# AI4Science-WestlakeU/RealPDEBench

Measured on AMD Instinct MI355X. Metric: train-step samples/sec (+ autoregressive rollout fields/sec in 'rollout'), FNO cylinder 128^2, higher is better.
Workload: dtype f32 storage / split-bf16x3 MFMA contractions (six bf16 products per fp32 product, fp32 accumulate), fp32-grade

## Files before the change

### realpdebench_amd/csrc/rpb_pjg.hip

```cpp
#include "rpb_pjf.h"
#include "rpb_mma.h"
#include <stdlib.h>

#define PG_HID 128
#define PG_WAVES 4
#define PG_GH_PLANE 2048
#define PG_GH_BUF (3 * PG_GH_PLANE)
#define PG_GH_WAVE (2 * PG_GH_BUF)
#ifndef PG_PIPE1
#define PG_PIPE1 2
#endif

#ifdef PG_TIMING
#define PG_T(i)                                    \
    {                                              \
        __builtin_amdgcn_sched_barrier(0);         \
        const long long now_ = clock64();          \
        __builtin_amdgcn_sched_barrier(0);         \
        tacc[i] += (float)(now_ - tlast);          \
        tlast = now_;                              \
    }
#else
#define PG_T(i)
#endif

#define PG_MAC6(NC, ACC, AH, AM, AL, BH, BM, BL) PG_MAC6F(NC, ACC, AH, AM, AL, BH, BM, BL, PG_NOTFIRST)
#define PG_NOTFIRST(c) false
#define PG_MAC6F(NC, ACC, AH, AM, AL, BH, BM, BL, FIRST)                               \
    _Pragma("unroll") for (int c_ = 0; c_ < NC; ++c_) ACC(c_) = mfma32b(AH(c_), BL(c_), FIRST(c_) ? f32x16{} : ACC(c_)); \
    _Pragma("unroll") for (int c_ = 0; c_ < NC; ++c_) ACC(c_) = mfma32b(AL(c_), BH(c_), ACC(c_)); \
    _Pragma("unroll") for (int c_ = 0; c_ < NC; ++c_) ACC(c_) = mfma32b(AM(c_), BM(c_), ACC(c_)); \
    _Pragma("unroll") for (int c_ = 0; c_ < NC; ++c_) ACC(c_) = mfma32b(AH(c_), BM(c_), ACC(c_)); \
    _Pragma("unroll") for (int c_ = 0; c_ < NC; ++c_) ACC(c_) = mfma32b(AM(c_), BH(c_), ACC(c_)); \
    _Pragma("unroll") for (int c_ = 0; c_ < NC; ++c_) ACC(c_) = mfma32b(AH(c_), BH(c_), ACC(c_));

template <bool LOSS>
__global__ __launch_bounds__(PG_WAVES * 64, 1) void pjg_kernel(PjfArgs p) {
    extern __shared__ u32x4 lds4[];
    u32x4* W1B = lds4;
    u32x4* W1D = W1B + 4 * 4 * 3 * 64;
    float* b1l = reinterpret_cast<float*>(W1D + 8 * 2 * 3 * 64);
    float* meanl = b1l + PG_HID;
    float* gball = meanl + 64;
    char* GHall = reinterpret_cast<char*>(gball + PG_WAVES * 64);
    const int tid = threadIdx.x, lane = tid & 63;
    const int wave = __builtin_amdgcn_readfirstlane(tid >> 6);
    const int n = lane & 31, hg = lane >> 5;
    for (int idx = tid; idx < 4 * 4 * 64; idx += blockDim.x) {
        const int l = idx & 63, nt = (idx >> 6) & 3, ks = idx >> 8;
        float v[8];
#pragma unroll
        for (int e = 0; e < 8; ++e) {
            const int c = 16 * ks + 8 * (l >> 5) + e;
            v[e] = p.w1[(32 * nt + (l & 31)) * 64 + c] * (p.xf.gamma[c] * p.xf.invstd[c]);
        }
        bf16x8 h, m, lo;
        split8(v, h, m, lo);
        W1B[((ks * 4 + nt) * 3 + 0) * 64 + l] = __builtin_bit_cast(u32x4, h);
        W1B[((ks * 4 + nt) * 3 + 1) * 64 + l] = __builtin_bit_cast(u32x4, m);
        W1B[((ks * 4 + nt) * 3 + 2) * 64 + l] = __builtin_bit_cast(u32x4, lo);
    }
    for (int idx = tid; idx < 8 * 2 * 64; idx += blockDim.x) {
        const int l = idx & 63, mt = (idx >> 6) & 1, ks3 = idx >> 7;
        float v[8];
#pragma unroll
        for (int e = 0; e < 8; ++e) v[e] = p.w1[(16 * ks3 + 8 * (l >> 5) + e) * 64 + 32 * mt + (l & 31)];
        bf16x8 h, m, lo;
        split8(v, h, m, lo);
        W1D[((ks3 * 2 + mt) * 3 + 0) * 64 + l] = __builtin_bit_cast(u32x4, h);
        W1D[((ks3 * 2 + mt) * 3 + 1) * 64 + l] = __builtin_bit_cast(u32x4, m);
        W1D[((ks3 * 2 + mt) * 3 + 2) * 64 + l] = __builtin_bit_cast(u32x4, lo);
    }
    for (int h = tid; h < PG_HID; h += blockDim.x) {
        float a = p.b1[h];
        for (int c = 0; c < 64; ++c) a = __builtin_fmaf(p.w1[h * 64 + c], p.xf.beta[c], a);
        b1l[h] = a;
    }
    if (tid < 64) meanl[tid] = p.xf.mean[tid];
    __syncthreads();

    const CropMap cm = p.cm;
    const long nslots = (long)gridDim.x * PG_WAVES;
    const long slot = (long)blockIdx.x * PG_WAVES + wave;
    const unsigned line_bytes = (unsigned)cm.Wp * 256u;
    const f32x4 z4 = {0.f, 0.f, 0.f, 0.f};

    {
        const long G = (long)p.B * cm.Tp * cm.Hp;
        for (long g = slot; g < G; g += nslots) {
            const int h = (int)(g % cm.Hp);
            const int t = (int)((g / cm.Hp) % cm.Tp);
            if (h < cm.H && t < cm.T) continue;
            const rsrc_t ro = make_rsrc(p.g + g * cm.Wp * 64, line_bytes);
            for (int off = lane * 16; off < (int)line_bytes; off += 1024) st16<0>(z4, ro, off);
        }
    }

    const long GL = (long)p.B * cm.T * cm.H;
    const int TQ = (cm.W + 31) >> 5;
    char* GHw = GHall + wave * PG_GH_WAVE;
    float* gb = gball + wave * 64;
    const float meanB0 = p.xf.mean[2 * n], meanB1 = p.xf.mean[2 * n + 1];
    float w2r[2][4], b1r[4];
#pragma unroll
    for (int nt = 0; nt < 4; ++nt) {
        b1r[nt] = b1l[32 * nt + n];
        w2r[0][nt] = p.w2[32 * nt + n];
        w2r[1][nt] = p.w2[PG_HID + 32 * nt + n];
    }
    const float b2y = LOSS ? p.b2[n & 1] : 0.f;
    const int celly = 8 * (n >> 3) + 4 * hg + ((n >> 1) & 3);
    const int cells = 8 * ((n >> 2) & 3) + 4 * (n >> 4) + (n & 3);
    const int ghw0 = n * 64 + (((2 * hg + 0) ^ ((n >> 1) & 3)) << 4), ghw1 = n * 64 + (((2 * hg + 1) ^ ((n >> 1) & 3)) << 4);
    int tro[2];
    {
        const int s16 = lane & 15, a = s16 >> 2, b = s16 & 3, gsel = (lane >> 4) & 1;
#pragma unroll
        for (int hf = 0; hf < 2; ++hf) {
            const int row = 8 * hg + 4 * hf + a;
            tro[hf] = row * 64 + (((2 * gsel + (b >> 1)) ^ ((row >> 1) & 3)) << 4) + (b & 1) * 8;
        }
    }
    const bool bit3 = (n >> 3) & 1, bit2 = (n >> 2) & 1, bit1 = (n >> 1) & 1, bit0 = n & 1;

    float dw2[2][4], db1[4], gacc = 0.f, lacc = 0.f;
    f32x16 accM[4][2];
#pragma unroll
    for (int t = 0; t < 4; ++t) {
        db1[t] = 0.f;
        dw2[0][t] = dw2[1][t] = 0.f;
#pragma unroll
        for (int c = 0; c < 2; ++c)
#pragma unroll
            for (int r = 0; r < 16; ++r) accM[t][c][r] = 0.f;
    }

    auto line_of = [&](int gl) {
        const unsigned h = (unsigned)gl % (unsigned)cm.H, r2 = (unsigned)gl / (unsigned)cm.H;
        return (int)(((r2 / (unsigned)cm.T) * cm.Tp + r2 % (unsigned)cm.T) * cm.Hp + h);
    };
    u32x4 xa[8];
    auto issue_xa = [&](int pl, int q) {
        const bool ok = pl >= 0;
        const rsrc_t rx = make_rsrc(p.s + (long)(ok ? pl : 0) * cm.Wp * 64, ok ? (unsigned)cm.W * 256u : 0u);
#pragma unroll
        for (int i = 0; i < 8; ++i) xa[i] = ld16<0>(rx, (32 * q + n) * 256 + (i >> 1) * 64 + hg * 32 + (i & 1) * 16);
    };
    auto prefetch = [&](int pl, int q) -> unsigned {
        const bool ok = pl >= 0;
        const rsrc_t rx = make_rsrc(p.s + (long)(ok ? pl : 0) * cm.Wp * 64, ok ? (unsigned)cm.W * 256u : 0u);
        return __builtin_amdgcn_raw_buffer_load_b32(rx, 32 * q * 256 + lane * 128, 0, 0);
    };
    issue_xa(slot < GL ? line_of((int)slot) : -1, 0);
#ifdef PG_TIMING
    float tacc[12];
#pragma unroll
    for (int i = 0; i < 12; ++i) tacc[i] = 0.f;
    long long tlast = clock64();
#endif
    for (long gl = slot; gl < GL; gl += nslots) {
        const int pl = line_of((int)gl);
        const int gln = gl + nslots < GL ? (int)(gl + nslots) : -1;
        const int pln = gln >= 0 ? line_of(gln) : -1;
        const rsrc_t ro = make_rsrc(p.g + (long)pl * cm.Wp * 64, line_bytes);
        const rsrc_t rxl = make_rsrc(p.s + (long)pl * cm.Wp * 64, (unsigned)cm.W * 256u);
        const rsrc_t rg = make_rsrc(p.gout + gl * cm.W * 2, (unsigned)cm.W * 8u);
        for (int q = 0; q < TQ; ++q) {
            asm volatile("" ::: "memory");
            const bool last = q + 1 == TQ;
            const int pn = last ? pln : pl, qn = last ? 0 : q + 1;
            const unsigned pf = prefetch(pn, qn);
            const float yv = buf_load_f32(rg, ((32 * q + celly) * 2 + (n & 1)) * 4, 0);
            f32x4 G4[8];
            if (!LOSS) {
#pragma unroll
                for (int k = 0; k < 8; ++k) G4[k] = __builtin_bit_cast(f32x4, ld16<0>(rg, (32 * q + 8 * (k >> 1) + 4 * hg + 2 * (k & 1)) * 8));
            }
            PG_T(0)
            f32x16 acc[4];
#pragma unroll
            for (int nt = 0; nt < 4; ++nt)
#pragma unroll
                for (int r = 0; r < 16; ++r) acc[nt][r] = 0.f;
            bf16x8 Ah[2], Am[2], Al[2], bh[2][4], bm[2][4], bl[2][4];
            auto prep = [&](int ks) {
                float v[8];
                const f32x4 x0 = __builtin_bit_cast(f32x4, xa[2 * ks]), x1 = __builtin_bit_cast(f32x4, xa[2 * ks + 1]);
                const f32x4 m0 = *reinterpret_cast<const f32x4*>(meanl + 16 * ks + 8 * hg), m1 = *reinterpret_cast<const f32x4*>(meanl + 16 * ks + 8 * hg + 4);
#pragma unroll
                for (int c = 0; c < 4; ++c) {
                    v[c] = x0[c] - m0[c];
                    v[4 + c] = x1[c] - m1[c];
                }
                split8(v, Ah[ks & 1], Am[ks & 1], Al[ks & 1]);
#pragma unroll
                for (int nt = 0; nt < 4; ++nt) {
                    bh[ks & 1][nt] = __builtin_bit_cast(bf16x8, W1B[((ks * 4 + nt) * 3 + 0) * 64 + lane]);
                    bm[ks & 1][nt] = __builtin_bit_cast(bf16x8, W1B[((ks * 4 + nt) * 3 + 1) * 64 + lane]);
                    bl[ks & 1][nt] = __builtin_bit_cast(bf16x8, W1B[((ks * 4 + nt) * 3 + 2) * 64 + lane]);
                }
            };
            prep(0);
#pragma unroll
            for (int ks = 0; ks < 4; ++ks) {
                if (ks < 3) prep(ks + 1);
#define PG_ACC(c) acc[c]
#define PG_AH(c) Ah[ks & 1]
#define PG_AM(c) Am[ks & 1]
#define PG_AL(c) Al[ks & 1]
#define PG_BH(c) bh[ks & 1][c]
#define PG_BM(c) bm[ks & 1][c]
#define PG_BL(c) bl[ks & 1][c]
#define PG_FIRST(c) (ks == 0)
                PG_MAC6F(4, PG_ACC, PG_AH, PG_AM, PG_AL, PG_BH, PG_BM, PG_BL, PG_FIRST)
#undef PG_FIRST
#undef PG_ACC
#undef PG_AH
#undef PG_AM
#undef PG_AL
#undef PG_BH
#undef PG_BM
#undef PG_BL
#if PG_PIPE1
                if (ks < 3) {
#pragma unroll
                    for (int i = 0; i < 24; ++i) {
                        __builtin_amdgcn_sched_group_barrier(0x008, 1, 0);
                        __builtin_amdgcn_sched_group_barrier(0x002, PG_PIPE1, 0);
                        if (i < 14) __builtin_amdgcn_sched_group_barrier(0x100, 1, 0);
                    }
                }
                __builtin_amdgcn_sched_barrier(0);
#endif
            }
            asm volatile("" ::"v"(pf));
            __builtin_amdgcn_sched_barrier(0);
            PG_T(1)
            f32x2 xr[16];
            auto issue_xr = [&]() {
#pragma unroll
                for (int i = 0; i < 16; ++i) xr[i] = ld8<0>(rxl, (32 * q + 16 * (i >> 3) + 8 * ((i >> 2) & 1) + 4 * hg + (i & 3)) * 256 + n * 8);
            };
            float VV[4][16];
            if (LOSS) {
                f32x2 pp[16];
#pragma unroll
                for (int i = 0; i < 16; ++i) pp[i] = pk2(0.f);
#pragma unroll
                for (int nt = 0; nt < 4; ++nt) {
                    const f32x2 wp = {w2r[0][nt], w2r[1][nt]};
#pragma unroll
                    for (int r = 0; r < 16; r += 4) {
                        f32x2 v, d, v2, d2;
                        gelu_both_as2x2(f32x2{acc[nt][r], acc[nt][r + 1]} + pk2(b1r[nt]), f32x2{acc[nt][r + 2], acc[nt][r + 3]} + pk2(b1r[nt]), v, v2, d, d2);
                        VV[nt][r] = v[0], VV[nt][r + 1] = v[1], VV[nt][r + 2] = v2[0], VV[nt][r + 3] = v2[1];
                        acc[nt][r] = d[0], acc[nt][r + 1] = d[1], acc[nt][r + 2] = d2[0], acc[nt][r + 3] = d2[1];
                        pp[r] = pk_fma(pk2(v[0]), wp, pp[r]);
                        pp[r + 1] = pk_fma(pk2(v[1]), wp, pp[r + 1]);
                        pp[r + 2] = pk_fma(pk2(v2[0]), wp, pp[r + 2]);
                        pp[r + 3] = pk_fma(pk2(v2[1]), wp, pp[r + 3]);
                    }
                }
                float po[32];
#pragma unroll
                for (int i = 0; i < 16; ++i) po[2 * i] = pp[i][0], po[2 * i + 1] = pp[i][1];
                PG_T(2)
                __builtin_amdgcn_sched_barrier(0);
                issue_xr();
                float q1[16], q2[8], q3[4], q4[2];
#pragma unroll
                for (int i = 0; i < 16; ++i) {
                    const u32x2 sw = __builtin_amdgcn_permlane16_swap(__builtin_bit_cast(unsigned, po[i]), __builtin_bit_cast(unsigned, po[i + 16]), false, false);
                    q1[i] = asf(sw[0]) + asf(sw[1]);
                }
#pragma unroll
                for (int i = 0; i < 8; ++i) q2[i] = dpp_add(bit3 ? q1[i + 8] : q1[i], bit3 ? q1[i] : q1[i + 8], 0);
#pragma unroll
                for (int i = 0; i < 4; ++i) q3[i] = dpp_add(bit2 ? q2[i + 4] : q2[i], bit2 ? q2[i] : q2[i + 4], 1);
#pragma unroll
                for (int i = 0; i < 2; ++i) q4[i] = dpp_add(bit1 ? q3[i + 2] : q3[i], bit1 ? q3[i] : q3[i + 2], 2);
                const float outv = dpp_add(bit0 ? q4[1] : q4[0], bit0 ? q4[0] : q4[1], 3) + b2y;
                const bool valid = 32 * q + celly < cm.W;
                const float diff = outv - yv;
                lacc += valid ? diff * diff : 0.f;
                const float gv = valid ? p.gscale * diff : 0.f;
                gacc += gv;
                gb[lane] = gv;
                __builtin_amdgcn_fence(__ATOMIC_RELEASE, "wavefront");
                __builtin_amdgcn_wave_barrier();
                __builtin_amdgcn_fence(__ATOMIC_ACQUIRE, "wavefront");
#pragma unroll
                for (int k = 0; k < 8; ++k) G4[k] = *reinterpret_cast<const f32x4*>(gb + 32 * hg + 4 * k);
            } else {
                gacc += yv;
#pragma unroll
                for (int nt = 0; nt < 4; ++nt)
#pragma unroll
                    for (int r = 0; r < 16; r += 4) {
                        f32x2 v, d, v2, d2;
                        gelu_both_as2x2(f32x2{acc[nt][r], acc[nt][r + 1]} + pk2(b1r[nt]), f32x2{acc[nt][r + 2], acc[nt][r + 3]} + pk2(b1r[nt]), v, v2, d, d2);
                        VV[nt][r] = v[0], VV[nt][r + 1] = v[1], VV[nt][r + 2] = v2[0], VV[nt][r + 3] = v2[1];
                        acc[nt][r] = d[0], acc[nt][r + 1] = d[1], acc[nt][r + 2] = d2[0], acc[nt][r + 3] = d2[1];
                    }
                __builtin_amdgcn_sched_barrier(0);
                issue_xr();
            }
            PG_T(3)
            {
                f32x2 dwp[4][2];
#pragma unroll
                for (int nt = 0; nt < 4; ++nt) {
                    dwp[nt][0] = f32x2{dw2[0][nt], dw2[1][nt]};
                    dwp[nt][1] = pk2(0.f);
                }
#pragma unroll
                for (int r = 0; r < 16; ++r)
#pragma unroll
                    for (int nt = 0; nt < 4; ++nt)
                        dwp[nt][r & 1] = pk_fma(f32x2{G4[r >> 1][2 * (r & 1)], G4[r >> 1][2 * (r & 1) + 1]}, pk2(VV[nt][r]), dwp[nt][r & 1]);
#pragma unroll
                for (int nt = 0; nt < 4; ++nt) {
                    const f32x2 t2 = dwp[nt][0] + dwp[nt][1];
                    dw2[0][nt] = t2[0], dw2[1][nt] = t2[1];
                }
            }
            PG_T(4)
            bf16x8 Xh[2][2], Xm[2][2], Xl[2][2];
#pragma unroll
            for (int kstep = 0; kstep < 2; ++kstep) {
                float v0[8], v1[8];
#pragma unroll
                for (int e = 0; e < 8; ++e) {
                    v0[e] = xr[8 * kstep + e][0] - meanB0;
                    v1[e] = xr[8 * kstep + e][1] - meanB1;
                }
                split8(v0, Xh[kstep][0], Xm[kstep][0], Xl[kstep][0]);
                split8(v1, Xh[kstep][1], Xm[kstep][1], Xl[kstep][1]);
            }
            __builtin_amdgcn_sched_barrier(0);
            PG_T(5)
            f32x16 acc3[2];
#pragma unroll
            for (int mt = 0; mt < 2; ++mt)
#pragma unroll
                for (int r = 0; r < 16; ++r) acc3[mt][r] = 0.f;
            bf16x8 Gh[2][2], Gm[2][2], Gl[2][2];
            auto gh_stage = [&](int nt) {
#pragma unroll
                for (int r = 0; r < 16; ++r) {
                    const float g0 = G4[r >> 1][2 * (r & 1)], g1 = G4[r >> 1][2 * (r & 1) + 1];
                    const float gp = __builtin_fmaf(g1, w2r[1][nt], g0 * w2r[0][nt]);
                    const float gh = gp * acc[nt][r];
                    acc[nt][r] = gh;
                    db1[nt] += gh;
                }
#pragma unroll
                for (int kstep = 0; kstep < 2; ++kstep) {
                    float v[8];
#pragma unroll
                    for (int e = 0; e < 8; ++e) v[e] = acc[nt][8 * kstep + e];
                    split8(v, Gh[nt & 1][kstep], Gm[nt & 1][kstep], Gl[nt & 1][kstep]);
                }
                char* ghb = GHw + (nt & 1) * PG_GH_BUF;
                *reinterpret_cast<u32x4*>(ghb + 0 * PG_GH_PLANE + ghw0) = __builtin_bit_cast(u32x4, Gh[nt & 1][0]);
                *reinterpret_cast<u32x4*>(ghb + 0 * PG_GH_PLANE + ghw1) = __builtin_bit_cast(u32x4, Gh[nt & 1][1]);
                *reinterpret_cast<u32x4*>(ghb + 1 * PG_GH_PLANE + ghw0) = __builtin_bit_cast(u32x4, Gm[nt & 1][0]);
                *reinterpret_cast<u32x4*>(ghb + 1 * PG_GH_PLANE + ghw1) = __builtin_bit_cast(u32x4, Gm[nt & 1][1]);
                *reinterpret_cast<u32x4*>(ghb + 2 * PG_GH_PLANE + ghw0) = __builtin_bit_cast(u32x4, Gl[nt & 1][0]);
                *reinterpret_cast<u32x4*>(ghb + 2 * PG_GH_PLANE + ghw1) = __builtin_bit_cast(u32x4, Gl[nt & 1][1]);
            };
            gh_stage(0);
            PG_T(6)
#pragma unroll
            for (int nt = 0; nt < 4; ++nt) {
                asm volatile("" ::: "memory");
                if (nt == 2) issue_xa(pn, qn);
                char* ghb = GHw + (nt & 1) * PG_GH_BUF;
                bf16x8 Bp[2][3], ah[2][2], am[2][2], al[2][2];
#pragma unroll
                for (int kk = 0; kk < 2; ++kk) {
#pragma unroll
                    for (int pln_ = 0; pln_ < 3; ++pln_) {
                        typedef bf16x4 __attribute__((address_space(3))) * lds_b4;
                        const bf16x4 lo = __builtin_amdgcn_ds_read_tr16_b64_v4bf16((lds_b4)(ghb + pln_ * PG_GH_PLANE + kk * 1024 + tro[0]));
                        const bf16x4 hi = __builtin_amdgcn_ds_read_tr16_b64_v4bf16((lds_b4)(ghb + pln_ * PG_GH_PLANE + kk * 1024 + tro[1]));
                        Bp[kk][pln_] = __builtin_shufflevector(lo, hi, 0, 1, 2, 3, 4, 5, 6, 7);
                    }
#pragma unroll
                    for (int mt = 0; mt < 2; ++mt) {
                        ah[kk][mt] = __builtin_bit_cast(bf16x8, W1D[(((2 * nt + kk) * 2 + mt) * 3 + 0) * 64 + lane]);
                        am[kk][mt] = __builtin_bit_cast(bf16x8, W1D[(((2 * nt + kk) * 2 + mt) * 3 + 1) * 64 + lane]);
                        al[kk][mt] = __builtin_bit_cast(bf16x8, W1D[(((2 * nt + kk) * 2 + mt) * 3 + 2) * 64 + lane]);
                    }
                }
                asm volatile("" ::: "memory");
#pragma unroll
                for (int kstep = 0; kstep < 2; ++kstep) {
#define PG_ACC(c) (*((c) < 2 ? &accM[nt][(c)] : &acc3[(c) - 2]))
#define PG_AH(c) ((c) < 2 ? Gh[nt & 1][kstep] : ah[kstep][(c) - 2])
#define PG_AM(c) ((c) < 2 ? Gm[nt & 1][kstep] : am[kstep][(c) - 2])
#define PG_AL(c) ((c) < 2 ? Gl[nt & 1][kstep] : al[kstep][(c) - 2])
#define PG_BH(c) ((c) < 2 ? Xh[kstep][(c)] : Bp[kstep][0])
#define PG_BM(c) ((c) < 2 ? Xm[kstep][(c)] : Bp[kstep][1])
#define PG_BL(c) ((c) < 2 ? Xl[kstep][(c)] : Bp[kstep][2])
#define PG_FIRST(c) ((c) >= 2 && nt == 0 && kstep == 0)
                    PG_MAC6F(4, PG_ACC, PG_AH, PG_AM, PG_AL, PG_BH, PG_BM, PG_BL, PG_FIRST)
#undef PG_FIRST
#undef PG_ACC
#undef PG_AH
#undef PG_AM
#undef PG_AL
#undef PG_BH
#undef PG_BM
#undef PG_BL
                }
                if (nt < 3) gh_stage(nt + 1);
                PG_T(8)
            }
            PG_T(9)
#pragma unroll
            for (int mt = 0; mt < 2; ++mt)
#pragma unroll
                for (int a = 0; a < 4; ++a) {
                    const f32x4 o = {acc3[mt][4 * a], acc3[mt][4 * a + 1], acc3[mt][4 * a + 2], acc3[mt][4 * a + 3]};
                    st16<0>(o, ro, (32 * q + cells) * 256 + (32 * mt + 8 * a + 4 * hg) * 4);
                }
        }
        PG_T(10)
        for (int off = TQ * 32 * 256 + lane * 16; off < (int)line_bytes; off += 1024) st16<0>(z4, ro, off);
    }

    if (LOSS) {
        const float ls = wave_sum(lacc);
        if (lane == 0) p.loss_part[slot] = ls;
    }
    float* part = p.part + slot * ((long)PG_HID * 64 + 2L * PG_HID + PG_HID + 2);
    {
        const float is0 = p.xf.invstd[2 * n], is1 = p.xf.invstd[2 * n + 1];
#pragma unroll
        for (int mt = 0; mt < 4; ++mt)
#pragma unroll
            for (int r = 0; r < 16; ++r) {
                const int h = 32 * mt + 8 * (r >> 2) + 4 * hg + (r & 3);
                float2 o;
                o.x = accM[mt][0][r] * is0;
                o.y = accM[mt][1][r] * is1;
                *reinterpret_cast<float2*>(part + h * 64 + 2 * n) = o;
            }
    }
#pragma unroll
    for (int nt = 0; nt < 4; ++nt) {
        float s1 = db1[nt];
        s1 += __shfl_xor(s1, 32, 64);
        if (hg == 0) part[PG_HID * 64 + 2 * PG_HID + 32 * nt + n] = s1;
#pragma unroll
        for (int j = 0; j < 2; ++j) {
            float s2 = dw2[j][nt];
            s2 += __shfl_xor(s2, 32, 64);
            if (hg == 0) part[PG_HID * 64 + j * PG_HID + 32 * nt + n] = s2;
        }
    }
#ifdef PG_TIMING
    if (lane < 12) {
        float tv = 0.f;
#pragma unroll
        for (int i = 0; i < 12; ++i) tv = lane == i ? tacc[i] : tv;
        part[lane] = tv;
    }
#endif
    {
        float s3 = gacc;
#pragma unroll
        for (int off = 2; off < 64; off <<= 1) s3 += __shfl_xor(s3, off, 64);
        if (lane < 2) part[PG_HID * 64 + 2 * PG_HID + PG_HID + lane] = s3;
    }
}

size_t pjg_lds() { return (size_t)(4 * 4 * 3 * 64 + 8 * 2 * 3 * 64) * 16 + (PG_HID + 64 + PG_WAVES * 64) * 4 + (size_t)PG_WAVES * PG_GH_WAVE; }

int pjg_supported(int DO) {
    return DO == 2;
}

int pjg_launch(PjfArgs& p, bool loss, int grid, hipStream_t st) {
    const size_t lds = pjg_lds();
    if (loss) {
        (void)hipFuncSetAttribute((const void*)pjg_kernel<true>, hipFuncAttributeMaxDynamicSharedMemorySize, (int)lds);
        hipLaunchKernelGGL((pjg_kernel<true>), dim3(grid), dim3(PG_WAVES * 64), lds, st, p);
    } else {
        (void)hipFuncSetAttribute((const void*)pjg_kernel<false>, hipFuncAttributeMaxDynamicSharedMemorySize, (int)lds);
        hipLaunchKernelGGL((pjg_kernel<false>), dim3(grid), dim3(PG_WAVES * 64), lds, st, p);
    }
    RPB_CHECK_LAUNCH("head_bwd");
}
```

Baseline: 888.6.

## Reuse split input from LDS via transposed reads instead of reloading from global

The already-split bf16 hi/mid/lo planes of the mean-centred input, computed for the first GEMM, are now stored to LDS. The weight-gradient GEMM reads them back with ds_read_tr16 transposed loads. This replaces the second global load of the input line and its second split, cutting global traffic and VALU work. In exchange it adds LDS stores interleaved into the MFMA schedule and reuses the GH LDS region. The layout of the weight-gradient output changes from channel-interleaved to channel-planar, with invstd indexing adjusted to match.

```diff
diff --git a/realpdebench_amd/csrc/rpb_pjg.hip b/realpdebench_amd/csrc/rpb_pjg.hip
--- a/realpdebench_amd/csrc/rpb_pjg.hip
+++ b/realpdebench_amd/csrc/rpb_pjg.hip
@@ -7,6 +7,7 @@
 #define PG_GH_PLANE 2048
 #define PG_GH_BUF (3 * PG_GH_PLANE)
 #define PG_GH_WAVE (2 * PG_GH_BUF)
+#define PG_SX_PLANE 4096
 #ifndef PG_PIPE1
 #define PG_PIPE1 2
 #endif
@@ -100,7 +101,6 @@
     const int TQ = (cm.W + 31) >> 5;
     char* GHw = GHall + wave * PG_GH_WAVE;
     float* gb = gball + wave * 64;
-    const float meanB0 = p.xf.mean[2 * n], meanB1 = p.xf.mean[2 * n + 1];
     float w2r[2][4], b1r[4];
 #pragma unroll
     for (int nt = 0; nt < 4; ++nt) {
@@ -120,6 +120,13 @@
             const int row = 8 * hg + 4 * hf + a;
             tro[hf] = row * 64 + (((2 * gsel + (b >> 1)) ^ ((row >> 1) & 3)) << 4) + (b & 1) * 8;
         }
+    }
+    const int sxw = n * 128 + ((hg << 4) ^ ((((n & 3) << 1) | ((n >> 2) & 1)) << 4));
+    int sxr[2];
+    {
+        const int s16 = lane & 15, a = s16 >> 2, b = s16 & 3, gsel = (lane >> 4) & 1;
+#pragma unroll
+        for (int ct = 0; ct < 2; ++ct) sxr[ct] = (4 * hg + a) * 128 + (((4 * ct + 2 * gsel + (b >> 1)) ^ ((a << 1) | hg)) << 4) + (b & 1) * 8;
     }
     const bool bit3 = (n >> 3) & 1, bit2 = (n >> 2) & 1, bit1 = (n >> 1) & 1, bit0 = n & 1;
 
@@ -163,7 +170,6 @@
         const int gln = gl + nslots < GL ? (int)(gl + nslots) : -1;
         const int pln = gln >= 0 ? line_of(gln) : -1;
         const rsrc_t ro = make_rsrc(p.g + (long)pl * cm.Wp * 64, line_bytes);
-        const rsrc_t rxl = make_rsrc(p.s + (long)pl * cm.Wp * 64, (unsigned)cm.W * 256u);
         const rsrc_t rg = make_rsrc(p.gout + gl * cm.W * 2, (unsigned)cm.W * 8u);
         for (int q = 0; q < TQ; ++q) {
             asm volatile("" ::: "memory");
@@ -199,6 +205,10 @@
                     bm[ks & 1][nt] = __builtin_bit_cast(bf16x8, W1B[((ks * 4 + nt) * 3 + 1) * 64 + lane]);
                     bl[ks & 1][nt] = __builtin_bit_cast(bf16x8, W1B[((ks * 4 + nt) * 3 + 2) * 64 + lane]);
                 }
+                char* sxb = GHw + (sxw ^ (ks << 5));
+                *reinterpret_cast<u32x4*>(sxb + 0 * PG_SX_PLANE) = __builtin_bit_cast(u32x4, Ah[ks & 1]);
+                *reinterpret_cast<u32x4*>(sxb + 1 * PG_SX_PLANE) = __builtin_bit_cast(u32x4, Am[ks & 1]);
+                *reinterpret_cast<u32x4*>(sxb + 2 * PG_SX_PLANE) = __builtin_bit_cast(u32x4, Al[ks & 1]);
             };
             prep(0);
 #pragma unroll
@@ -228,6 +238,7 @@
                         __builtin_amdgcn_sched_group_barrier(0x008, 1, 0);
                         __builtin_amdgcn_sched_group_barrier(0x002, PG_PIPE1, 0);
                         if (i < 14) __builtin_amdgcn_sched_group_barrier(0x100, 1, 0);
+                        if (i >= 21) __builtin_amdgcn_sched_group_barrier(0x200, 1, 0);
                     }
                 }
                 __builtin_amdgcn_sched_barrier(0);
@@ -236,11 +247,6 @@
             asm volatile("" ::"v"(pf));
             __builtin_amdgcn_sched_barrier(0);
             PG_T(1)
-            f32x2 xr[16];
-            auto issue_xr = [&]() {
-#pragma unroll
-                for (int i = 0; i < 16; ++i) xr[i] = ld8<0>(rxl, (32 * q + 16 * (i >> 3) + 8 * ((i >> 2) & 1) + 4 * hg + (i & 3)) * 256 + n * 8);
-            };
             float VV[4][16];
             if (LOSS) {
                 f32x2 pp[16];
@@ -266,7 +272,6 @@
                 for (int i = 0; i < 16; ++i) po[2 * i] = pp[i][0], po[2 * i + 1] = pp[i][1];
                 PG_T(2)
                 __builtin_amdgcn_sched_barrier(0);
-                issue_xr();
                 float q1[16], q2[8], q3[4], q4[2];
 #pragma unroll
                 for (int i = 0; i < 16; ++i) {
@@ -303,7 +308,6 @@
                         acc[nt][r] = d[0], acc[nt][r + 1] = d[1], acc[nt][r + 2] = d2[0], acc[nt][r + 3] = d2[1];
                     }
                 __builtin_amdgcn_sched_barrier(0);
-                issue_xr();
             }
             PG_T(3)
             {
@@ -326,17 +330,22 @@
             }
             PG_T(4)
             bf16x8 Xh[2][2], Xm[2][2], Xl[2][2];
-#pragma unroll
-            for (int kstep = 0; kstep < 2; ++kstep) {
-                float v0[8], v1[8];
-#pragma unroll
-                for (int e = 0; e < 8; ++e) {
-                    v0[e] = xr[8 * kstep + e][0] - meanB0;
-                    v1[e] = xr[8 * kstep + e][1] - meanB1;
-                }
-                split8(v0, Xh[kstep][0], Xm[kstep][0], Xl[kstep][0]);
-                split8(v1, Xh[kstep][1], Xm[kstep][1], Xl[kstep][1]);
-            }
+            asm volatile("" ::: "memory");
+#pragma unroll
+            for (int kstep = 0; kstep < 2; ++kstep)
+#pragma unroll
+                for (int ct = 0; ct < 2; ++ct) {
+                    typedef bf16x4 __attribute__((address_space(3))) * lds_b4;
+                    bf16x8 xp[3];
+#pragma unroll
+                    for (int pln_ = 0; pln_ < 3; ++pln_) {
+                        const bf16x4 lo = __builtin_amdgcn_ds_read_tr16_b64_v4bf16((lds_b4)(GHw + pln_ * PG_SX_PLANE + kstep * 2048 + sxr[ct]));
+                        const bf16x4 hi = __builtin_amdgcn_ds_read_tr16_b64_v4bf16((lds_b4)(GHw + pln_ * PG_SX_PLANE + kstep * 2048 + 1024 + sxr[ct]));
+                        xp[pln_] = __builtin_shufflevector(lo, hi, 0, 1, 2, 3, 4, 5, 6, 7);
+                    }
+                    Xh[kstep][ct] = xp[0], Xm[kstep][ct] = xp[1], Xl[kstep][ct] = xp[2];
+                }
+            asm volatile("" ::: "memory");
             __builtin_amdgcn_sched_barrier(0);
             PG_T(5)
             f32x16 acc3[2];
@@ -436,16 +445,14 @@
     }
     float* part = p.part + slot * ((long)PG_HID * 64 + 2L * PG_HID + PG_HID + 2);
     {
-        const float is0 = p.xf.invstd[2 * n], is1 = p.xf.invstd[2 * n + 1];
+        const float is0 = p.xf.invstd[n], is1 = p.xf.invstd[32 + n];
 #pragma unroll
         for (int mt = 0; mt < 4; ++mt)
 #pragma unroll
             for (int r = 0; r < 16; ++r) {
                 const int h = 32 * mt + 8 * (r >> 2) + 4 * hg + (r & 3);
-                float2 o;
-                o.x = accM[mt][0][r] * is0;
-                o.y = accM[mt][1][r] * is1;
-                *reinterpret_cast<float2*>(part + h * 64 + 2 * n) = o;
+                part[h * 64 + n] = accM[mt][0][r] * is0;
+                part[h * 64 + 32 + n] = accM[mt][1][r] * is1;
             }
     }
 #pragma unroll
```

Result: no change. 893.0 (median of 6 runs) (+0.5%).
